# DanHelmy/hdr-realtime-video-pipeline

Hardware: AMD Instinct MI355X
Metric: frames/sec (HDRTVNet++ AGCM+LE+HG fp16 3840x2160 + fused RGB48 post into the pinned host ring); p50 per-frame ms in p50_ms (higher is better)
Workload: dtype f16

## Files before the change

### hdr-realtime-video-pipeline_amd/csrc/api_graph.hip

```cpp
#include "api.h"

namespace hdrtv_host {

void Seq::conv(const std::string &key, const f16 *src0, int c0, const f16 *src1, int c1, int Hi, int Wi, int act, int mode, f16 *dst, int dstC, int Hd, int Wd, const f16 *res1, const f16 *res2, f16 *dst_full, f16 *dst_planar, const f16 *res_planar, const float *dotw, float *dst_dot, int s0_stride)
{
    if (!ok()) return;
    auto it = c->conv.find(key);
    if (it == c->conv.end()) { rc = fail(c, HDRTV_ESTATE, "no packed conv %s", key.c_str()); return; }
    const ConvLayer &L = it->second;
    ConvParams p;
    memset(&p, 0, sizeof p);
    p.src0 = src0; p.src1 = src1; p.c0 = c0; p.c1 = c1;
    p.s0_stride = s0_stride ? s0_stride : c0; p.s1_stride = c1;
    p.Hi = Hi; p.Wi = Wi;
    const int pad = L.ks / 2;
    p.Ho = (Hi + 2 * pad - L.ks) / L.stride + 1;
    p.Wo = (Wi + 2 * pad - L.ks) / L.stride + 1;
    p.wpk = wtp<f16>(c, L.wpk); p.scale = wtp<float>(c, L.scale); p.shift = wtp<float>(c, L.shift);
    p.CoutPad = L.coutPad; p.Cout = L.cout; p.act = act; p.mode = mode;
    p.dst = dst; p.dst_full = dst_full; p.dstC = dstC; p.Hd = Hd; p.Wd = Wd;
    p.res1 = res1; p.res2 = res2; p.dst_planar = dst_planar; p.res_planar = res_planar;
    p.dotw = dotw; p.dst_dot = dst_dot;
    if (c0 + c1 != L.cin) { rc = fail(c, HDRTV_ESTATE, "conv %s: channel mismatch", key.c_str()); return; }
    p.zeros = wtp<f16>(c, c->zeros_off);
// ... 473 lines not shown
                q.chk(conv_c3_q8_launch(img, H, W, wtp<int8_t>(c, Lq.wpk8), wtp<float>(c, Lq.scale), wtp<float>(c, Lq.shift), Lq.q.inv(),
                                        Lq.q.zoff(), ACT_RELU, f0a, c->n_cu, q.s),
                      "LE.conv_first", "conv_c3_q8", (double)H * W * 27 * 32, (double)H * W * (6.0 + 64.0));
            }
            q.conv32("LE.HR_conv1", f0a, cond1, "LE.SFT_layer1", H, W, ACT_RELU, ST_NHWC, fea0, 32, H, W);
        } else {
            const bool fuse = !c->var.at("no_c3fuse") && !c->var.at("conv32_old") && c->q32.find("LE.HR_conv1") == c->q32.end();
            if (fuse) {
                q.conv32("LE.HR_conv1", f0a, cond1, "LE.SFT_layer1", H, W, ACT_RELU, ST_NHWC, fea0, 32, H, W, nullptr, nullptr, nullptr, nullptr,
                         img, "le.conv_first");
            } else {
                q.c3("le.conv_first", img, H, W, ACT_RELU, f0a, nullptr);
                q.conv32("LE.HR_conv1", f0a, cond1, "LE.SFT_layer1", H, W, ACT_RELU, ST_NHWC, fea0, 32, H, W);
            }
        }
    }
    f16 *fea1a = q.wsp<f16>("le.fea1a"), *fea1 = q.wsp<f16>("le.fea1"), *l1b = q.wsp<f16>("le.l1b");
    auto down = [&](const char *key, const f16 *src, int Hi, int Wi, f16 *dst, int Ho, int Wo) {
        if (isq8(key)) q.convq8(key, src, false, 32, Hi, Wi, ACT_RELU, dst, 32, nullptr);
        else q.conv(key, src, 32, nullptr, 0, Hi, Wi, ACT_RELU, ST_NHWC, dst, 32, Ho, Wo);
    };
    if (!head_fused) down("LE.down_conv1", fea0, H, W, fea1a, s.H1, s.W1);
    q.resblock("LE.recon_trunk1.0", fea1a, cond2, s.H1, s.W1, l1b, fea1);
    f16 *fea2a = q.wsp<f16>("le.fea2a"), *fea2 = q.wsp<f16>("le.fea2"), *l2b = q.wsp<f16>("le.l2b");
    down("LE.down_conv2", fea1, s.H1, s.W1, fea2a, s.H2, s.W2);
    q.resblock("LE.recon_trunk2.0", fea2a, cond3, s.H2, s.W2, l2b, fea2);
    f16 *fea3 = q.wsp<f16>("le.fea3"), *l3b = q.wsp<f16>("le.l3b"), *t3x = q.wsp<f16>("le.t3x"), *t3y = q.wsp<f16>("le.t3y");
    down("LE.down_conv3", fea2, s.H2, s.W2, fea3, s.H3, s.W3);
    q.resblock("LE.recon_trunk3.0", fea3, cond4, s.H3, s.W3, l3b, t3x);
    q.resblock("LE.recon_trunk3.1", t3x, cond4, s.H3, s.W3, l3b, t3y);
    q.resblock("LE.recon_trunk3.2", t3y, cond4, s.H3, s.W3, l3b, t3x);
    q.resblock("LE.recon_trunk3.3", t3x, cond4, s.H3, s.W3, l3b, t3y, fea3);
    f16 *up1 = q.wsp<f16>("le.up1"), *t4 = q.wsp<f16>("le.t4");
    q.conv32("LE.up_conv1.0", t3y, nullptr, "", s.H3, s.W3, ACT_RELU, ST_PS, up1, 32, s.H2, s.W2, fea2);
    q.resblock("LE.recon_trunk4.0", up1, cond3, s.H2, s.W2, l2b, t4);
    f16 *up2 = q.wsp<f16>("le.up2"), *t5 = q.wsp<f16>("le.t5");
    q.conv32("LE.up_conv2.0", t4, nullptr, "", s.H2, s.W2, ACT_RELU, ST_PS, up2, 32, s.H1, s.W1, fea1);
    q.resblock("LE.recon_trunk5.0", up2, cond2, s.H1, s.W1, l1b, t5);
    if (q.ok() && rows && c->var.at("le_rows_i8")) {
        auto qu = c->q32.find("LE.up_conv3.0"), qh = c->q32.find("LE.HR_conv2"), ql = c->q32.find("LE.conv_last");
        const SftLayer &S2 = c->sft.at("LE.SFT_layer2");
        if (qu != c->q32.end() && qh != c->q32.end() && ql != c->q32.end() && S2.q && qu->second.coutPad == 128 &&
            qh->second.coutPad == 32 && ql->second.coutPad == 32) {
            RowsTailI8Params p;
            memset(&p, 0, sizeof p);
            p.u = t5; p.fea0 = fea0; p.cond = cond1; p.res_planar = img; p.dst_planar = out_planar; p.H = H; p.W = W;
            p.up = q.rows_i8(qu->second); p.hr = q.rows_i8(qh->second); p.last = q.rows_i8(ql->second); p.s = q.rows_i8(S2);
            p.slope_relu = act_slope(ACT_RELU);
            p.trash = const_cast<char *>(wtp<char>(c, c->dump_off));
            const double npx = (double)H * W;
            q.chk(le_tail_rows_i8_launch(p, c->n_cu, q.s), "LE.tail", "le_tail_rows<i8>",
                  npx * (32.0 * 9 * 128 / 4 + 2.0 * (16 * 16 + 16 * 32) + 32.0 * 9 * 32 + 32.0 * 9 * 3), npx * (16 + 64 + 32 + 6 + 6) + 9.0 * 32 * (128 + 32 + 32));
            return q.rc;
        }
    }
    if (q.ok() && rows) {
        RowsTailParams p;
        memset(&p, 0, sizeof p);
        bool qu, qh, ql, qs;
        const ConvLayer *Lu = q.rows_conv("LE.up_conv3.0", p.fq_u, qu), *Lh = q.rows_conv("LE.HR_conv2", p.fq_y, qh),
                        *Ll = q.rows_conv("LE.conv_last", p.fq_z, ql);
        const SftLayer &S2 = c->sft.at("LE.SFT_layer2");
        if (Lu && Lh && Ll && q.rows_sft(S2, p.fq_s, qs)) {
            p.fq = (qu ? 1 : 0) | (qh ? 2 : 0) | (ql ? 4 : 0) | (qs ? 8 : 0);
            p.u = t5; p.fea0 = fea0; p.cond = cond1; p.res_planar = img; p.dst_planar = out_planar; p.H = H; p.W = W;
            p.w_up = wtp<f16>(c, Lu->wpk); p.b_up = wtp<float>(c, Lu->shift);
            p.sft_wfrag = wtp<f16>(c, S2.wfrag); p.sft_bias = wtp<float>(c, S2.bias);
            p.w_hr = wtp<f16>(c, Lh->wpk); p.b_hr = wtp<float>(c, Lh->shift); p.w_last = wtp<f16>(c, Ll->wpk); p.b_last = wtp<float>(c, Ll->shift);
            p.trash = const_cast<char *>(wtp<char>(c, c->dump_off));
            p.dump = q.stamp_buf();
            const double npx = (double)H * W;
            q.chk(le_tail_rows_launch(p, c->n_cu, q.s), "LE.tail", p.fq ? "le_tail_rows<fq>" : "le_tail_rows",
                  npx * (32.0 * 9 * 128 / 4 + 2.0 * (16 * 16 + 16 * 32) + 32.0 * 9 * 32 + 32.0 * 9 * 3), npx * (16 + 64 + 32 + 6 + 6) + 2.0 * 9 * 32 * (128 + 32 + 32));
            return q.rc;
        }
    }
    q.conv32("LE.up_conv3.0", t5, nullptr, "", s.H1, s.W1, ACT_RELU, ST_PS, up3, 32, H, W, fea0);
    q.conv32("LE.HR_conv2", up3, cond1, "LE.SFT_layer2", H, W, ACT_RELU, ST_NHWC, f0b, 32, H, W);
    q.conv32("LE.conv_last", f0b, nullptr, "", H, W, ACT_NONE, ST_PLANAR3, nullptr, 0, H, W, nullptr, nullptr, out_planar, img);
    return q.rc;
}

size_t hg_need_plan(hdrtv_ctx *c, int Hp, int Wp, HgNeedParams &p)
{
    memset(&p, 0, sizeof p);
    p.Hp = Hp; p.Wp = Wp;
    constexpr int n_layers = (int)(sizeof hg_layers / sizeof hg_layers[0]);
    static_assert(n_layers + 1 <= HG_NEED_MAX_LAYERS && n_layers + 3 <= HG_NEED_MAX_TENSORS, "hg_need's tables are too small");
    constexpr int max_level = [] { int m = 0; for (const HgLayer &L : hg_layers) m = L.level > m ? L.level : m; return m; }();
    static_assert(max_level < HG_NEED_LEVELS, "hg_need's unit tables have too few levels");
    memcpy(p.lu, hg_need_unit_log2[c->var.at("hg_sparse") == 1 ? 1 : 2], sizeof p.lu);
    auto ncell = [&](int level) { return (((Hp >> level) + 15) / 16) * (((Wp >> level) + 15) / 16); };
    auto nwords = [&](int level) {
        size_t m = 0;
        for (const auto &tab : hg_need_unit_log2) {
            const int u = 1 << tab[level], rows = std::max(((Hp >> level) + u - 1) / u, ((Hp >> level) + 7) / 8);
            m = std::max(m, (size_t)rows * ((((Wp >> level) + u - 1) / u + 63) / 64));
        }
        return m;
    };
    const char *names[HG_NEED_MAX_TENSORS];
    int level[HG_NEED_MAX_TENSORS], nt = 0;
    auto tensor = [&](const char *name, int lev) {
        if (!name) name = "part";
        for (int i = 0; i < nt; ++i)
            if (!strcmp(names[i], name)) return i;
        names[nt] = name; level[nt] = lev;
        return nt++;
    };
    for (int i = 0; i < n_layers; ++i) {
        const HgLayer &L = hg_layers[i];
        HgNeedLayer &N = p.L[i + 1];
        N.level = L.level; N.ks = L.ks; N.tw = 16;
        N.mode = L.mode == ST_POOL ? 1 : (L.ps ? 2 : 0);
        N.in = tensor(L.in, L.level);
        N.skip = L.skip ? tensor(L.skip, L.level) : -1;
        N.out = tensor(L.out, L.out_level());
        N.th = L.ks == 3 && Seq::prw_tile_rows(c, L.mode, L.cout, Hp >> L.level, Wp >> L.level) == 8 ? 8 : 16;
    }
    const int nt_table = nt;
    {
        HgNeedLayer &N = p.L[0];
        N.level = 0; N.ks = 3; N.mode = 1;
        N.out = tensor(hg_layers[0].in, 1);
        N.in = tensor("img", 0);
        N.skip = -1;
        N.th = 8; N.tw = 32;
    }
    p.n_layers = n_layers + 1;
    bool seen[HG_NEED_MAX_TENSORS] = {};
    for (int i = p.n_layers - 1; i >= 0; --i) {
        HgNeedLayer &N = p.L[i];
        N.in_first = !seen[N.in];
        seen[N.in] = true;
        if (N.skip >= 0) { N.skip_first = !seen[N.skip]; seen[N.skip] = true; }
    }
    size_t off = 0;
    auto take = [&](size_t bytes) { const size_t o = off; off = (off + bytes + 15) & ~(size_t)15; return (int)o; };
    p.flags_off = take((size_t)ncell(0));
    take((size_t)ncell(0));
    for (int t = 0; t < nt_table; ++t)
        if (strcmp(names[t], "part")) take((size_t)ncell(level[t]));
    for (int i = 1; i <= n_layers; ++i) p.L[i].list_off = take(4 * (2 * (size_t)ncell(p.L[i].level) + 4));
    size_t scratch = 0;
    for (int t = 0; t < nt; ++t) scratch = std::max(scratch, nwords(level[t]));
    for (int t = 0; t < nt_table; ++t) {
        p.map_off[t] = take(8 * nwords(level[t]));
        if (!strcmp(names[t], "part")) p.flags_map = t;
    }
    for (int i = 0; i < p.n_layers; ++i) {
        p.L[i].out_chained = i + 1 < p.n_layers ? p.L[i + 1].in == p.L[i].out : p.L[i].out == p.flags_map;
        p.L[i].in_chained = i > 0 && p.L[i - 1].out == p.L[i].in;
    }
    p.scratch_words = (int)scratch;
    p.kbits_off = take(8 * scratch);
    p.tbits_off = take(8 * scratch);
    p.L[0].list_off = take(4 * (2 * (size_t)ncell(0) + 4));
    p.map_off[nt_table] = take(8 * nwords(0));
    return off;
}

int run_hg(hdrtv_ctx *c, Seq &q, const f16 *base, void *out, int out_f32, bool complete_taps)
{
    const Shapes s = shapes_for(c->H, c->W);
    const int Hp = s.Hp, Wp = s.Wp;
    f16 *img = q.wsp<f16>("hg.img");
    uint8_t *mask = q.wsp<uint8_t>("hg.mask");
    const bool sparse = !complete_taps && c->var.at("hg_sparse") != 0 && !c->hg_i8 && !c->var.at("final_recompute");
    HgNeedParams np;
    if (sparse) {
        hg_need_plan(c, Hp, Wp, np);
        np.base = q.wsp<unsigned char>("hg.need");
    }
    if (q.ws == c->lane_ws[0] && !complete_taps) {
        hipStreamCaptureStatus cap = hipStreamCaptureStatusNone;
        c->taps_partial = sparse;
        c->taps_replayable = sparse && hipStreamIsCapturing(q.s, &cap) == hipSuccess && cap != hipStreamCaptureStatusNone;
        c->taps_stream = q.s;
    }
    if (!complete_taps)
        q.chk(hg_prep_launch(base, s.H, s.W, Hp, Wp, img, mask, c->mask_r, 0.1f, q.s, sparse ? np.base + np.flags_off : nullptr), "hg_prep",
              "hg_prep", 0.0, 13.0 * Hp * Wp);
    if (sparse) q.chk(hg_need_launch(np, q.s), "hg_need", "hg_need", 0.0, 0.0);
    float *part = q.wsp<float>("hg.part");
    const bool light = !c->var.at("final_recompute");
    float *part2 = light ? q.wsp<float>("hg.part2") : nullptr;
    const f16 *w2frag = light ? wtp<f16>(c, c->hgf_wfrag) + 6 * 64 * 8 : nullptr;
    constexpr int n_layers = (int)(sizeof hg_layers / sizeof hg_layers[0]);
    const char *tn[3 * n_layers];
    void *tp[3 * n_layers];
    int nt = 0;
    auto tensor = [&](const char *name) -> void * {
        if (!name) return nullptr;
        for (int i = 0; i < nt; ++i)
            if (!strcmp(tn[i], name)) return tp[i];
        char key[32];
        snprintf(key, sizeof key, "%s%s", c->hg_i8 ? "hg8." : "hg.", name);
        tn[nt] = name;
        tp[nt] = q.wsp<void>(key);
        return tp[nt++];
    };
    const bool c1_list = sparse && light;
    q.c3("hg.conv1", img, Hp, Wp, ACT_RELU, nullptr, (f16 *)tensor(hg_layers[0].in), c->hg_q0_inv, c->hg_q0_zero, w2frag, part2,
         c1_list ? reinterpret_cast<const int *>(np.base + np.L[0].list_off) : nullptr, c1_list ? ((Hp + 7) / 8) * ((Wp + 31) / 32) : 0);
    char key[32];
    for (const HgLayer &L : hg_layers) {
        snprintf(key, sizeof key, "hg.%s", L.name);
        if (sparse) {
            const HgNeedLayer &N = np.L[&L - hg_layers + 1];
            q.need_list = reinterpret_cast<const int *>(np.base + N.list_off);
            q.need_th = N.th;
            q.need_total = (((Hp >> L.level) + N.th - 1) / N.th) * (((Wp >> L.level) + 15) / 16);
        }
        const int c1 = L.skip_cin, c0 = L.cin - c1, Hi = Hp >> L.level, Wi = Wp >> L.level;
        const int Ho = Hp >> L.out_level(), Wo = Wp >> L.out_level();
        const bool dot3 = L.mode == ST_PS_DOT3;
        const float *dotw = dot3 ? wtp<float>(c, c->hg_w10a) : nullptr;
        float *dst_dot = dot3 ? part : nullptr;
        if (c->hg_i8)
            q.conv8(key, (const int8_t *)tensor(L.in), c0, (const int8_t *)tensor(L.skip), c1, Hi, Wi, L.mode, tensor(L.out), L.out_c(), Ho, Wo, dotw, dst_dot);
        else
            q.conv(key, (const f16 *)tensor(L.in), c0, (const f16 *)tensor(L.skip), c1, Hi, Wi, L.act, L.mode, (f16 *)tensor(L.out), L.out_c(), Ho, Wo,
                   nullptr, nullptr, nullptr, nullptr, nullptr, dotw, dst_dot);
    }
    if (!q.ok() || complete_taps) return q.rc;
    const C3Layer &L1 = c->c3.at("hg.conv1");
    HgFinalFusedArgs fa;
    fa.img = img; fa.mask = mask; fa.part = part; fa.wfrag = wtp<f16>(c, c->hgf_wfrag);
    fa.scale = wtp<float>(c, L1.scale); fa.shift = wtp<float>(c, L1.shift);
    fa.b10 = wtp<float>(c, c->f32v.at("hg.b10"));
    fa.wl = wtp<float>(c, c->f32v.at("hg.wl")); fa.bl = wtp<float>(c, c->f32v.at("hg.bl"));
    fa.out = out; fa.out_f32 = out_f32; fa.H = s.H; fa.W = s.W; fa.Hp = Hp; fa.Wp = Wp;
    if (light)
        q.chk(hg_final_light_launch(fa, part2, q.s), "hg_final", "hg_final_light", (double)s.H * s.W * 6 * 3,
              (double)s.H * s.W * (6 + 1 + 32 + 3 * (out_f32 ? 4 : 2)));
#ifdef HDRTV_AB
    else
        q.chk(hg_final_fused_launch(fa, c->n_cu, q.s), "hg_final", "hg_final_fused", (double)Hp * Wp * (128 * 3 + 6 * 3),
              (double)s.H * s.W * (6 + 1 + 16 + 3 * (out_f32 ? 4 : 2)));
#endif
    return q.rc;
}

}
```

### hdr-realtime-video-pipeline_amd/csrc/api_util.hip

```cpp
#include "api.h"

namespace hdrtv_host {

int fail(hdrtv_ctx *c, int code, const char *fmt, ...)
{
    char buf[512];
    va_list ap;
    va_start(ap, fmt);
    vsnprintf(buf, sizeof buf, fmt, ap);
    va_end(ap);
    if (c) { std::lock_guard<std::mutex> lk(c->err_mu); c->err = buf; }
    return code;
}

namespace {
const std::pair<const char *, int> k_variants[] = {
    {"le_rows", 1},
    {"le_rows_min", 8},
    {"le_rows_i8", 1},
    {"le_rows_fq", 1},
    {"prw", 1},
    {"prw_i8", 1},
    {"pglds_nt_slow", 3},
    {"no_t16", 0},
    {"conv32_old", 0},
    {"conv32_nosplit", 0},
    {"conv32_nw", 0},
    {"no_c3fuse", 0},
    {"no_c3q8", 0},
    {"glds1_old", 0},
    {"hg_sparse", 2},
    {"final_recompute", 0},
    {"cond3_fused", 1},
    {"cond2_fused", 1},
    {"pre_split", 0},
    {"force_ncu", 0},
    {"light_wgs", 2},
    {"fs_passes", 3},
    {"f32_narrow_below", 0},
    {"f32_mfma", 1},
};
const char *const k_ab_only[] = {"conv32_old", "conv32_nosplit", "conv32_nw", "glds1_old", "final_recompute"};
}
bool variant_allowed(const std::string &name, int value)
{
#ifdef HDRTV_AB
    (void)name; (void)value;
    return true;
#else
    if (value == 0) return true;
    for (const char *n : k_ab_only) if (name == n) return false;
    return true;
#endif
}
void variants_init(hdrtv_ctx *c)
{
    for (const auto &kv : k_variants) c->var[kv.first] = kv.second;
    const char *e = getenv("HDRTV_VARIANTS");
    if (!e) return;
    std::string str(e);
    size_t pos = 0;
    while (pos < str.size()) {
        size_t nx = str.find(',', pos);
        if (nx == std::string::npos) nx = str.size();
        const std::string one = str.substr(pos, nx - pos);
        const size_t eq = one.find('=');
        if (eq != std::string::npos) {
            auto it = c->var.find(one.substr(0, eq));
            if (it != c->var.end() && variant_allowed(it->first, atoi(one.c_str() + eq + 1))) it->second = atoi(one.c_str() + eq + 1);
        }
        pos = nx + 1;
    }
}

}
```

### hdr-realtime-video-pipeline_amd/csrc/hg_need.hip

```cpp
#include "launchers.h"

namespace {

constexpr int NT = 1024, LDS_WORDS = 2304;
using u64 = unsigned long long;

__constant__ u64 k_tile_bits[5] = {~0ull, 0x5555555555555555ull, 0x1111111111111111ull, 0x0101010101010101ull, 0x0001000100010001ull};

struct Map {
    int h, w, nw;
};
__device__ __forceinline__ Map map_of(const HgNeedParams &p, int level)
{
    const int lu = p.lu[level], r = (1 << lu) - 1;
    Map m;
    m.h = ((p.Hp >> level) + r) >> lu;
    m.w = ((p.Wp >> level) + r) >> lu;
    m.nw = (m.w + 63) >> 6;
    return m;
}
__device__ __forceinline__ u64 word(const u64 *b, const Map &m, int y, int wi)
{
    return (unsigned)y < (unsigned)m.h && (unsigned)wi < (unsigned)m.nw ? b[y * m.nw + wi] : 0;
}
__device__ __forceinline__ u64 row_mask(int w, int wi)
{
    const int n = w - 64 * wi;
    return n >= 64 ? ~0ull : (n <= 0 ? 0ull : (1ull << n) - 1);
}
__device__ __forceinline__ u64 spread2(unsigned v)
{
    u64 x = v;
    x = (x | x << 16) & 0x0000FFFF0000FFFFull;
    x = (x | x << 8) & 0x00FF00FF00FF00FFull;
    x = (x | x << 4) & 0x0F0F0F0F0F0F0F0Full;
    x = (x | x << 2) & 0x3333333333333333ull;
    x = (x | x << 1) & 0x5555555555555555ull;
    return x | x << 1;
}
__device__ __forceinline__ unsigned pairs_any(u64 v)
{
    u64 x = (v | v >> 1) & 0x5555555555555555ull;
    x = (x | x >> 1) & 0x3333333333333333ull;
    x = (x | x >> 2) & 0x0F0F0F0F0F0F0F0Full;
    x = (x | x >> 4) & 0x00FF00FF00FF00FFull;
    x = (x | x >> 8) & 0x0000FFFF0000FFFFull;
    x = (x | x >> 16) & 0x00000000FFFFFFFFull;
    return (unsigned)x;
}

__global__ __launch_bounds__(NT) void hg_need_kernel(HgNeedParams p)
{
    __shared__ u64 s_k[LDS_WORDS], s_t[LDS_WORDS], s_n[LDS_WORDS];
    __shared__ int s_wave[NT / 64];
    const int tid = threadIdx.x;
    {
        const Map m = map_of(p, 0);
        const HgNeedLayer &L = p.L[p.n_layers - 1];
        u64 *fb = L.out_chained && m.h * m.nw <= LDS_WORDS ? s_n : reinterpret_cast<u64 *>(p.base + p.map_off[p.flags_map]);
        unsigned char *fl = p.base + p.flags_off;
        constexpr int NW = NT / 64, B = 8;
        const int lane = tid & 63, n0 = m.h * m.nw;
        for (int i0 = tid >> 6; i0 < n0; i0 += B * NW) {
            int at[B];
            unsigned char c[B];
#pragma unroll
            for (int j = 0; j < B; ++j) {
                const int i = i0 + j * NW, y = i / m.nw, x = 64 * (i - y * m.nw) + lane;
                at[j] = i < n0 && x < m.w ? y * m.w + x : -1;
                c[j] = at[j] >= 0 ? fl[at[j]] : 0;
            }
#pragma unroll
            for (int j = 0; j < B; ++j) {
                const u64 v = __ballot(c[j] != 0);
                if (at[j] >= 0) fl[at[j]] = 0;
                if (lane == 0 && i0 + j * NW < n0) fb[i0 + j * NW] = v;
            }
        }
    }
    __syncthreads();
    for (int li = p.n_layers - 1; li >= 0; --li) {
        const HgNeedLayer L = p.L[li];
        const int olev = L.level + (L.mode == 1 ? 1 : 0) - (L.mode == 2 ? 1 : 0);
        const Map mk = map_of(p, L.level), mo = map_of(p, olev);
        const int lu = p.lu[L.level], nk = mk.h * mk.nw;
        const int sh = p.lu[olev] - lu + olev - L.level;
        const int lth = L.th == 8 ? 3 : 4, ltw = L.tw == 32 ? 5 : 4, lbw = ltw - lu;
        const int ty_n = ((p.Hp >> L.level) + L.th - 1) >> lth, tx_n = ((p.Wp >> L.level) + (1 << ltw) - 1) >> ltw, nt = ty_n * mk.nw;
        const bool lds = max(nk, nt) <= LDS_WORDS;
        u64 *km = lds ? s_k : reinterpret_cast<u64 *>(p.base + p.kbits_off);
        u64 *tm = lds ? s_t : reinterpret_cast<u64 *>(p.base + p.tbits_off);
        const u64 *om = L.out_chained && mo.h * mo.nw <= LDS_WORDS ? s_n : reinterpret_cast<const u64 *>(p.base + p.map_off[L.out]);
        for (int i = tid; i < nk; i += NT) {
            const int y = i / mk.nw, wi = i - y * mk.nw;
            u64 k;
            if (sh == 0) {
                k = word(om, mo, y, wi);
            } else if (sh > 0) {
                k = spread2((unsigned)(word(om, mo, y >> 1, wi >> 1) >> (32 * (wi & 1))));
            } else {
                k = 0;
                for (int dy = 0; dy < 2; ++dy)
                    k |= (u64)pairs_any(word(om, mo, 2 * y + dy, 2 * wi)) | (u64)pairs_any(word(om, mo, 2 * y + dy, 2 * wi + 1)) << 32;
            }
            km[i] = k & row_mask(mk.w, wi);
        }
        __syncthreads();
        u64 *ig = reinterpret_cast<u64 *>(p.base + p.map_off[L.in]), *im = L.in_chained && nk <= LDS_WORDS ? s_n : ig;
        u64 *sm = L.skip >= 0 ? reinterpret_cast<u64 *>(p.base + p.map_off[L.skip]) : nullptr;
        for (int i = tid; i < nk; i += NT) {
            const int y = i / mk.nw, wi = i - y * mk.nw;
            u64 v = km[i];
            if (L.ks == 3) {
                for (int dy = -1; dy <= 1; ++dy) {
                    const u64 c = word(km, mk, y + dy, wi);
                    v |= c | c << 1 | c >> 1 | word(km, mk, y + dy, wi - 1) >> 63 | word(km, mk, y + dy, wi + 1) << 63;
                }
                v &= row_mask(mk.w, wi);
            }
            im[i] = L.in_first ? v : (ig[i] | v);
            if (sm) sm[i] = L.skip_first ? v : (sm[i] | v);
        }
        const int r_sh = lth - lu;
        for (int i = tid; i < nt; i += NT) {
            const int ty = i / mk.nw, wi = i - ty * mk.nw;
            const int r0 = r_sh >= 0 ? ty << r_sh : ty >> -r_sh, nr = r_sh >= 0 ? 1 << r_sh : 1;
            u64 v = 0;
            for (int r = r0; r < min(r0 + nr, mk.h); ++r) v |= km[r * mk.nw + wi];
            for (int s = 1; s < (1 << lbw); s <<= 1) v |= v >> s;
            tm[i] = v & k_tile_bits[lbw];
        }
        __syncthreads();
        const int per = (nt + NT - 1) / NT, c0 = tid * per, c1 = min(nt, c0 + per);
        int cnt = 0;
        for (int i = c0; i < c1; ++i) cnt += __popcll(tm[i]);
        int incl = cnt;
        for (int d = 1; d < 64; d <<= 1) {
            const int v = __shfl_up(incl, d, 64);
            if ((tid & 63) >= d) incl += v;
        }
        if ((tid & 63) == 63) s_wave[tid >> 6] = incl;
        __syncthreads();
        int o = incl - cnt, total = 0;
        for (int w = 0; w < NT / 64; ++w) {
            const int v = s_wave[w];
            if (w < (tid >> 6)) o += v;
            total += v;
        }
        int *lst = reinterpret_cast<int *>(p.base + L.list_off);
        if (tid == 0) lst[0] = total;
        for (int i = c0; i < c1; ++i) {
            const int ty = i / mk.nw, wi = i - ty * mk.nw;
            for (u64 v = tm[i]; v; v &= v - 1) lst[1 + o++] = ty * tx_n + ((64 * wi + __ffsll(v) - 1) >> lbw);
        }
    }
}

}

hipError_t hg_need_launch(const HgNeedParams &p, hipStream_t s)
{
    if (!p.base || p.n_layers < 1 || p.n_layers > HG_NEED_MAX_LAYERS) return hipErrorInvalidValue;
    for (int i = 0; i < p.n_layers; ++i) {
        const HgNeedLayer &L = p.L[i];
        const int olev = L.level + (L.mode == 1 ? 1 : 0) - (L.mode == 2 ? 1 : 0);
        if (L.level < 0 || L.level >= HG_NEED_LEVELS || olev < 0 || olev >= HG_NEED_LEVELS) return hipErrorInvalidValue;
        const int sh = p.lu[olev] - p.lu[L.level] + olev - L.level;
        if (p.lu[L.level] < 0 || p.lu[L.level] > 4 || sh < -1 || sh > 1 || (L.th != 8 && L.th != 16) ||
            (L.tw != 0 && L.tw != 16 && L.tw != 32))
            return hipErrorInvalidValue;
    }
    if (p.lu[0] != 4) return hipErrorInvalidValue;
    hipLaunchKernelGGL(hg_need_kernel, dim3(1), dim3(NT), 0, s, p);
    return hipGetLastError();
}
```

### hdr-realtime-video-pipeline_amd/csrc/launchers.h

```cpp
#pragma once
#include "common.h"

struct DevOnce {
    unsigned char set[64] = {};
    static int cur() { int d = 0; return hipGetDevice(&d) == hipSuccess && d >= 0 && d < 64 ? d : 0; }
    bool need() const { return !set[cur()]; }
    void done() { set[cur()] = 1; }
};
template <class K> hipError_t allow_lds(DevOnce &once, K kern, int bytes)
{
    if (!once.need()) return hipSuccess;
    const hipError_t e = hipFuncSetAttribute(reinterpret_cast<const void *>(kern), hipFuncAttributeMaxDynamicSharedMemorySize, bytes);
    if (e == hipSuccess) once.done();
    return e;
}

hipError_t conv_igemm_launch(ConvParams p, int cin_t, int bn, int ks, int stride, hipStream_t stream);
hipError_t conv_glds1_launch(ConvParams p, hipStream_t stream, int n_cu = 0, bool old_form = false, bool *list_taken = nullptr);
hipError_t conv_pglds_launch(ConvParams p, int n_cu, hipStream_t stream, bool *list_taken = nullptr);
hipError_t conv_prw_launch(ConvParams p, int th, int n_cu, hipStream_t stream, bool *list_taken = nullptr);
hipError_t conv_pglds_i8_launch(ConvI8Params p, int n_cu, hipStream_t stream);
hipError_t conv_prw_i8_launch(ConvI8Params p, int th, int n_cu, hipStream_t stream);
hipError_t conv1x1_i8_launch(ConvI8Params p, hipStream_t stream);
hipError_t conv32p_launch(Conv32Params p, int n_cu, hipStream_t stream, int nw = 0);
hipError_t conv32s_launch(Conv32Params p, int n_cu, hipStream_t stream, bool nosplit = false);
hipError_t le_rb_rows_launch(RowsRbParams p, int n_cu, hipStream_t stream);
hipError_t le_rb_rows_i8_launch(RowsRbI8Params p, int n_cu, hipStream_t stream);
hipError_t le_tail_rows_i8_launch(RowsTailI8Params p, int n_cu, hipStream_t stream);
hipError_t le_head_rows_i8_launch(RowsHeadI8Params p, int n_cu, hipStream_t stream);
hipError_t le_tail_rows_launch(RowsTailParams p, int n_cu, hipStream_t stream);
hipError_t le_head_rows_launch(RowsHeadParams p, int n_cu, hipStream_t stream);
hipError_t conv_t16_launch(ConvParams p, hipStream_t stream, int n_cu);
hipError_t conv_q8_launch(ConvQ8Params p, hipStream_t stream, int n_cu);
hipError_t conv_q8_multi_launch(ConvQ8MultiParams p, int n_cu, hipStream_t stream);
hipError_t conv3x3s2_preg_launch(ConvParams p, int n_cu, hipStream_t stream);

hipError_t pre_unpack_launch(const uint8_t *bgr, f16 *out, int H, int W, hipStream_t s);
struct AaTables {
    const float *wx;
    const int *xmn, *xns;
    const float *wy;
    const int *ymn, *yns;
};
hipError_t cond_resize_launch(const f16 *in, f16 *out, int H, int W, int Ho, int Wo, const AaTables &t, hipStream_t s);
hipError_t pre_fused_launch(const uint8_t *bgr, f16 *out, f16 *cond, int H, int W, int Ho, int Wo, const AaTables &t, int mode, hipStream_t s);
hipError_t post_u8_launch(const void *in, int is_f32, int H, int W, uint8_t *bgr, hipStream_t s);
hipError_t post_rgb48_launch(const void *in, int is_f32, int H, int W, uint16_t *rgb, int pq, float peak, hipStream_t s,
                             const float *pq_bnd = nullptr);

struct FakeQ { int on; float inv, zoff, scale, zero; };
hipError_t cls_block_launch(const void *in, int in_f16, int Ci, int Hi, int Wi, const float *nmean, const float *nrstd,
                            const float *ngamma, const float *nbeta, const float *Wt, const float *bias, int Co, float *out,
                            int Ho, int Wo, float *part, hipStream_t s, const FakeQ *qin = nullptr, const FakeQ *qstat = nullptr,
                            int *nblk = nullptr);
hipError_t cls_stats_launch(const float *part, int C, int nblk, int n, float eps, float *mean, float *rstd, hipStream_t s);
struct AgcmFoldArgs {
    const float *mean5;
    const float *w20, *b20;
    const float *ws[3], *bs[3], *wt[3], *bt[3];
    const float *w1, *b1, *w2, *b2, *w3, *b3;
};
hipError_t agcm_fold_launch(const AgcmFoldArgs &a, f16 *frags, float *biasbuf, hipStream_t s);
hipError_t agcm_mlp_launch(const f16 *in, f16 *out, size_t npix, const f16 *frags, const float *biasbuf, hipStream_t s);

hipError_t conv_c3_launch(const f16 *in, int H, int W, const f16 *wfrag, const float *scale, const float *shift, int cout,
                          int act, f16 *out, f16 *out_pool, int n_cu, hipStream_t s, float pool_q_inv = 0.f, float pool_q_zero = 0.f,
                          const f16 *w2frag = nullptr, float *part2 = nullptr,
                          const int *tile_list = nullptr, bool *list_taken = nullptr);
hipError_t conv_c3_q8_launch(const f16 *in, int H, int W, const int8_t *wq, const float *scale, const float *shift, float q_inv,
                             float q_zoff, int act, f16 *out, int n_cu, hipStream_t s);
struct QLastArgs {
    const int8_t *wq;
    const float *ss;
    float q_inv, q_zoff;
};
hipError_t le_cond_trunk_launch(const f16 *img, int H, int W, const f16 *wfrag, const float *bias, f16 *cond, f16 *cond1,
                                int n_cu, hipStream_t s, const QLastArgs *q6 = nullptr);
hipError_t cond_tail_launch(const f16 *x, int x_stride, size_t npx, const f16 *wfrag, const float *bias, f16 *out, int n_cu,
                            hipStream_t s, const QLastArgs *q2 = nullptr);
struct TrunkQ8Args {
    const int8_t *wfrag;
    const float *consts;
    float q1_inv, q1_zoff, q4_inv;
    float zoff[5];
};
hipError_t le_cond_trunk_q8_launch(const f16 *img, int H, int W, const TrunkQ8Args &a, f16 *cond, f16 *cond1, int n_cu, hipStream_t s);
hipError_t cond_tail_q8_launch(const int8_t *x, size_t npx, const int8_t *wfrag, const float *consts, float zoff2, f16 *out, int n_cu,
                               hipStream_t s);
hipError_t agcm_mlp_q8_launch(const f16 *in, f16 *out, size_t npix, const int8_t *wfrag, const float *consts, float q1_inv, float q1_zoff,
                              float zoff2, float zoff3, hipStream_t s);
hipError_t planar3_to_q8_launch(const f16 *in, size_t npix, float inv, float zoff, int8_t *out, hipStream_t s);
struct AgcmFoldQ8Args {
    FakeQ q20, qlin[6];
    const float *P, *Q;
    float inv2, inv3;
    float *consts;
};
hipError_t agcm_fold_q8_launch(const AgcmFoldArgs &a, const AgcmFoldQ8Args &q, float *biasbuf, hipStream_t s);
hipError_t hg_prep_launch(const f16 *base, int H, int W, int Hp, int Wp, f16 *img_pad, uint8_t *mask, float r, float thresh,
                          hipStream_t s, uint8_t *flags = nullptr);
constexpr int HG_NEED_MAX_LAYERS = 24, HG_NEED_MAX_TENSORS = 32, HG_NEED_LEVELS = 6;
constexpr int hg_need_unit_log2[3][HG_NEED_LEVELS] = {{4, 4, 4, 4, 4, 4}, {4, 4, 4, 4, 4, 4}, {4, 2, 1, 0, 0, 0}};
struct HgNeedLayer {
    int level, mode, ks;
    int in, skip, out;
    int in_first, skip_first;
    int out_chained;
    int in_chained;
    int th, tw;
    int list_off;
};
struct HgNeedParams {
    unsigned char *base;
    int Hp, Wp, n_layers;
    int lu[HG_NEED_LEVELS];
    int flags_off;
    int flags_map;
    int kbits_off, tbits_off, scratch_words;
    int map_off[HG_NEED_MAX_TENSORS];
    HgNeedLayer L[HG_NEED_MAX_LAYERS];
};
hipError_t hg_need_launch(const HgNeedParams &p, hipStream_t s);
struct HgFinalFusedArgs {
    const f16 *img;
    const uint8_t *mask;
    const float *part;
    const f16 *wfrag;
    const float *scale, *shift, *b10, *wl, *bl;
    void *out;
    int out_f32, H, W, Hp, Wp;
};
hipError_t hg_final_fused_launch(const HgFinalFusedArgs &a, int n_cu, hipStream_t s);
hipError_t hg_final_light_launch(const HgFinalFusedArgs &a, const float *part2, hipStream_t s);
hipError_t letterbox_launch(const LetterboxParams &p, hipStream_t s);
hipError_t post_scale_launch(const PostScaleParams &p, int is_f32, int pq, hipStream_t s);
hipError_t post_scale_ar_launch(const PostScaleParams &p, int antiring, int is_f32, int pq, hipStream_t s);
hipError_t post_scale_cas_launch(const PostScaleParams &p, int antiring, int cas, int is_f32, int pq, hipStream_t s);
hipError_t post_fsr_launch(const PostFsrParams &p, int rcas, float sharp, int is_f32, int pq, hipStream_t s);
hipError_t film_grain_launch(const uint16_t *src, uint16_t *dst, int H, int W, float intensity, float seed, hipStream_t s);
hipError_t post_rgb48_grain_launch(const void *in, int is_f32, int H, int W, uint16_t *rgb, int pq, float peak, const float *pq_bnd,
                                   float intensity, float seed, hipStream_t s);
hipError_t post_scale_grain_launch(const PostScaleParams &p, int antiring, int cas, float intensity, float seed, int is_f32, int pq,
                                   hipStream_t s);
hipError_t post_fsr_grain_launch(const PostFsrParams &p, int rcas, float sharp, float intensity, float seed, int is_f32, int pq, hipStream_t s);
hipError_t post_down_launch(const PostDownParams &p, int antiring, int ssim, int is_f32, int pq, hipStream_t s);
hipError_t post_ssimsr_launch(const PostSsimsrParams &p, int ssim, int is_f32, int pq, hipStream_t s);
hipError_t post_ycbcr10_launch(const Ycbcr10Params &p, int is_f32, int pq, hipStream_t s);
hipError_t rgb48_to_ycbcr10_launch(const Ycbcr10Params &p, hipStream_t s);
hipError_t post_ycbcr10_dither_launch(const Ycbcr10Params &p, int is_f32, int pq, hipStream_t s);
hipError_t rgb48_to_ycbcr10_dither_launch(const Ycbcr10Params &p, hipStream_t s);
int64_t ycbcr10_fs_scratch_bytes(int fmt, int H, int W);
hipError_t post_ycbcr10_fs_launch(const Ycbcr10Params &p, int is_f32, int pq, void *scratch, int passes, hipStream_t s);
hipError_t rgb48_to_ycbcr10_fs_launch(const Ycbcr10Params &p, void *scratch, int passes, hipStream_t s);
hipError_t rgb48_deband_launch(const DebandParams &p, hipStream_t s);
hipError_t light_stats_launch(const LightStatsParams &p, int is_f32, int pq, int max_wgs, hipStream_t s);
hipError_t rgb48_light_stats_launch(const LightStatsParams &p, int max_wgs, hipStream_t s);
hipError_t metrics_launch(const MetricsParams &p, hipStream_t s);
int metrics_blocks(int H, int W);
hipError_t metrics_u16_launch(const MetricsParams &p, hipStream_t s);
hipError_t border_counts_launch(const BorderCountsParams &p, hipStream_t s);
bool area_reduce_size_ok(int sh, int sw, int nh, int nw);
hipError_t area_reduce_launch(const AreaReduceParams &p, hipStream_t s);
hipError_t channel_hist_launch(const ChannelHistParams &p, hipStream_t s);
void grade_match_host(const uint32_t *hist, double n, float peak_nits, float *out12);

hipError_t conv_f32_launch(const F32ConvParams &p, int ks, int stride, int n_cu, hipStream_t s);
bool conv_f32_on_mfma(const F32ConvParams &p, int ks, int n_cu);
hipError_t ew_f32_launch(int op, const float *a, const float *b, const float *c, float *y, size_t n, hipStream_t s);
hipError_t avgpool3s2_leaky_f32_launch(const float *x, float *y, int C, int H, int W, float slope, hipStream_t s);
hipError_t instnorm_f32_launch(float *x, const float *gamma, const float *beta, int C, int n, float eps, hipStream_t s);
hipError_t plane_mean_f32_launch(const float *x, float *y, int C, int n, hipStream_t s);
hipError_t gfm_heads_f32_launch(const F32GfmParams &p, hipStream_t s);
hipError_t maxpool2_f32_launch(const float *x, float *y, int C, int H, int W, hipStream_t s);
hipError_t window_f32_launch(const float *x, float *y, int C, int H, int W, int Ho, int Wo, int mode, hipStream_t s);
hipError_t hg_mask_f32_launch(const float *base, float *mask, size_t npix, float r, hipStream_t s);
hipError_t hg_blend_f32_launch(const float *t, const float *img, const float *mask, float *out, int H, int W, int Hp, int Wp,
                               hipStream_t s);
hipError_t pre_f32_launch(const uint8_t *bgr, float *rgb, float *cond, int H, int W, int Ho, int Wo, const AaTables &t, int mode, hipStream_t s);
hipError_t cond_resize_f32_launch(const float *rgb, float *cond, int H, int W, int Ho, int Wo, const AaTables &t, int mode, hipStream_t s);
```

Baseline: 149.5.

## Speed up HG need-planning kernel with LDS-resident maps and early exits

Rewrites the single-workgroup hg_need kernel so that, when every layer's bitmaps fit, all maps including skip maps stay in LDS, using lighter barriers. Adds fast paths: return immediately when no flags are set, and stop propagating when a layer's need mask is full, emitting dense tile lists for the remaining layers. The list compaction changes from a per-thread serial scan to wave-parallel ballot-based emission, and the flag gather runs with larger unrolling. This targets the latency of a serial one-block planning kernel, at the cost of more complexity and more LDS.

```diff
diff --git a/hdr-realtime-video-pipeline_amd/csrc/api_graph.hip b/hdr-realtime-video-pipeline_amd/csrc/api_graph.hip
--- a/hdr-realtime-video-pipeline_amd/csrc/api_graph.hip
+++ b/hdr-realtime-video-pipeline_amd/csrc/api_graph.hip
@@ -649,6 +649,7 @@
         p.L[i].out_chained = i + 1 < p.n_layers ? p.L[i + 1].in == p.L[i].out : p.L[i].out == p.flags_map;
         p.L[i].in_chained = i > 0 && p.L[i - 1].out == p.L[i].in;
     }
+    p.fast = c->var.at("hg_need_fast") != 0;
     p.scratch_words = (int)scratch;
     p.kbits_off = take(8 * scratch);
     p.tbits_off = take(8 * scratch);
diff --git a/hdr-realtime-video-pipeline_amd/csrc/api_util.hip b/hdr-realtime-video-pipeline_amd/csrc/api_util.hip
--- a/hdr-realtime-video-pipeline_amd/csrc/api_util.hip
+++ b/hdr-realtime-video-pipeline_amd/csrc/api_util.hip
@@ -30,6 +30,7 @@
     {"no_c3q8", 0},
     {"glds1_old", 0},
     {"hg_sparse", 2},
+    {"hg_need_fast", 1},
     {"final_recompute", 0},
     {"cond3_fused", 1},
     {"cond2_fused", 1},
diff --git a/hdr-realtime-video-pipeline_amd/csrc/hg_need.hip b/hdr-realtime-video-pipeline_amd/csrc/hg_need.hip
--- a/hdr-realtime-video-pipeline_amd/csrc/hg_need.hip
+++ b/hdr-realtime-video-pipeline_amd/csrc/hg_need.hip
@@ -2,7 +2,8 @@
 
 namespace {
 
-constexpr int NT = 1024, LDS_WORDS = 2304;
+constexpr int NT = 1024, NWAVE = NT / 64, LDS_WORDS = 2304, SKIP_SLOTS = 4;
+constexpr int LDS_BYTES = 3 * LDS_WORDS * 8, LDS_BYTES_ALL = (3 + SKIP_SLOTS) * LDS_WORDS * 8;
 using u64 = unsigned long long;
 
 __constant__ u64 k_tile_bits[5] = {~0ull, 0x5555555555555555ull, 0x1111111111111111ull, 0x0101010101010101ull, 0x0001000100010001ull};
@@ -10,7 +11,7 @@
 struct Map {
     int h, w, nw;
 };
-__device__ __forceinline__ Map map_of(const HgNeedParams &p, int level)
+__host__ __device__ __forceinline__ Map map_of(const HgNeedParams &p, int level)
 {
     const int lu = p.lu[level], r = (1 << lu) - 1;
     Map m;
@@ -18,6 +19,19 @@
     m.w = ((p.Wp >> level) + r) >> lu;
     m.nw = (m.w + 63) >> 6;
     return m;
+}
+__host__ __device__ __forceinline__ int out_level(const HgNeedLayer &L) { return L.level + (L.mode == 1 ? 1 : 0) - (L.mode == 2 ? 1 : 0); }
+struct Tiles {
+    int lth, ltw, ty_n, tx_n;
+};
+__host__ __device__ __forceinline__ Tiles tiles_of(const HgNeedParams &p, const HgNeedLayer &L)
+{
+    Tiles t;
+    t.lth = L.th == 8 ? 3 : 4;
+    t.ltw = L.tw == 32 ? 5 : 4;
+    t.ty_n = ((p.Hp >> L.level) + L.th - 1) >> t.lth;
+    t.tx_n = ((p.Wp >> L.level) + (1 << t.ltw) - 1) >> t.ltw;
+    return t;
 }
 __device__ __forceinline__ u64 word(const u64 *b, const Map &m, int y, int wi)
 {
@@ -48,49 +62,74 @@
     x = (x | x >> 16) & 0x00000000FFFFFFFFull;
     return (unsigned)x;
 }
-
-__global__ __launch_bounds__(NT) void hg_need_kernel(HgNeedParams p)
-{
-    __shared__ u64 s_k[LDS_WORDS], s_t[LDS_WORDS], s_n[LDS_WORDS];
-    __shared__ int s_wave[NT / 64];
-    const int tid = threadIdx.x;
+template <bool ALL> __device__ __forceinline__ void chain_barrier()
+{
+    if constexpr (ALL) {
+        __builtin_amdgcn_fence(__ATOMIC_RELEASE, "workgroup", "local");
+        __builtin_amdgcn_s_barrier();
+        __builtin_amdgcn_fence(__ATOMIC_ACQUIRE, "workgroup", "local");
+    } else {
+        __syncthreads();
+    }
+}
+
+template <bool ALL> __global__ __launch_bounds__(NT) void hg_need_kernel(HgNeedParams p)
+{
+    extern __shared__ u64 s_maps[];
+    u64 *const s_k = s_maps, *const s_t = s_maps + LDS_WORDS, *const s_n = s_maps + 2 * LDS_WORDS, *const s_skip = s_maps + 3 * LDS_WORDS;
+    __shared__ int s_wave[NWAVE], s_any[NWAVE], s_full[NWAVE];
+    const int tid = threadIdx.x, lane = tid & 63, wave = tid >> 6;
     {
         const Map m = map_of(p, 0);
         const HgNeedLayer &L = p.L[p.n_layers - 1];
-        u64 *fb = L.out_chained && m.h * m.nw <= LDS_WORDS ? s_n : reinterpret_cast<u64 *>(p.base + p.map_off[p.flags_map]);
+        u64 *fb = ALL || (L.out_chained && m.h * m.nw <= LDS_WORDS) ? s_n : reinterpret_cast<u64 *>(p.base + p.map_off[p.flags_map]);
         unsigned char *fl = p.base + p.flags_off;
-        constexpr int NW = NT / 64, B = 8;
-        const int lane = tid & 63, n0 = m.h * m.nw;
-        for (int i0 = tid >> 6; i0 < n0; i0 += B * NW) {
+        constexpr int B = 16;
+        const int n0 = m.h * m.nw;
+        u64 any = 0;
+        for (int i0 = wave; i0 < n0; i0 += B * NWAVE) {
             int at[B];
             unsigned char c[B];
 #pragma unroll
             for (int j = 0; j < B; ++j) {
-                const int i = i0 + j * NW, y = i / m.nw, x = 64 * (i - y * m.nw) + lane;
+                const int i = i0 + j * NWAVE, y = i / m.nw, x = 64 * (i - y * m.nw) + lane;
                 at[j] = i < n0 && x < m.w ? y * m.w + x : -1;
-                c[j] = at[j] >= 0 ? fl[at[j]] : 0;
+                c[j] = fl[max(at[j], 0)];
             }
 #pragma unroll
             for (int j = 0; j < B; ++j) {
-                const u64 v = __ballot(c[j] != 0);
+                const u64 v = __ballot(at[j] >= 0 && c[j] != 0);
+                any |= v;
                 if (at[j] >= 0) fl[at[j]] = 0;
-                if (lane == 0 && i0 + j * NW < n0) fb[i0 + j * NW] = v;
-            }
-        }
-    }
-    __syncthreads();
-    for (int li = p.n_layers - 1; li >= 0; --li) {
+                if (lane == 0 && i0 + j * NWAVE < n0) fb[i0 + j * NWAVE] = v;
+            }
+        }
+        if (lane == 0) s_any[wave] = any != 0;
+    }
+    chain_barrier<ALL>();
+    if (p.fast) {
+        int any = 0;
+        for (int w = 0; w < NWAVE; ++w) any |= s_any[w];
+        if (!any) {
+            if (tid == 0)
+                for (int l = 0; l < p.n_layers; ++l) *reinterpret_cast<int *>(p.base + p.L[l].list_off) = 0;
+            return;
+        }
+    }
+    int li = p.n_layers - 1;
+    for (; li >= 0; --li) {
         const HgNeedLayer L = p.L[li];
-        const int olev = L.level + (L.mode == 1 ? 1 : 0) - (L.mode == 2 ? 1 : 0);
+        const int olev = out_level(L);
         const Map mk = map_of(p, L.level), mo = map_of(p, olev);
         const int lu = p.lu[L.level], nk = mk.h * mk.nw;
         const int sh = p.lu[olev] - lu + olev - L.level;
-        const int lth = L.th == 8 ? 3 : 4, ltw = L.tw == 32 ? 5 : 4, lbw = ltw - lu;
-        const int ty_n = ((p.Hp >> L.level) + L.th - 1) >> lth, tx_n = ((p.Wp >> L.level) + (1 << ltw) - 1) >> ltw, nt = ty_n * mk.nw;
-        const bool lds = max(nk, nt) <= LDS_WORDS;
+        const Tiles T = tiles_of(p, L);
+        const int lth = T.lth, lbw = T.ltw - lu, ty_n = T.ty_n, tx_n = T.tx_n, nt = ty_n * mk.nw;
+        const bool lds = ALL || max(nk, nt) <= LDS_WORDS;
         u64 *km = lds ? s_k : reinterpret_cast<u64 *>(p.base + p.kbits_off);
         u64 *tm = lds ? s_t : reinterpret_cast<u64 *>(p.base + p.tbits_off);
-        const u64 *om = L.out_chained && mo.h * mo.nw <= LDS_WORDS ? s_n : reinterpret_cast<const u64 *>(p.base + p.map_off[L.out]);
+        const u64 *om = ALL || (L.out_chained && mo.h * mo.nw <= LDS_WORDS) ? s_n : reinterpret_cast<const u64 *>(p.base + p.map_off[L.out]);
+        bool full = true;
         for (int i = tid; i < nk; i += NT) {
             const int y = i / mk.nw, wi = i - y * mk.nw;
             u64 k;
@@ -103,11 +142,24 @@
                 for (int dy = 0; dy < 2; ++dy)
                     k |= (u64)pairs_any(word(om, mo, 2 * y + dy, 2 * wi)) | (u64)pairs_any(word(om, mo, 2 * y + dy, 2 * wi + 1)) << 32;
             }
-            km[i] = k & row_mask(mk.w, wi);
-        }
-        __syncthreads();
-        u64 *ig = reinterpret_cast<u64 *>(p.base + p.map_off[L.in]), *im = L.in_chained && nk <= LDS_WORDS ? s_n : ig;
-        u64 *sm = L.skip >= 0 ? reinterpret_cast<u64 *>(p.base + p.map_off[L.skip]) : nullptr;
+            const u64 rm = row_mask(mk.w, wi);
+            km[i] = k & rm;
+            full = full && (k & rm) == rm;
+        }
+        {
+            const u64 not_full = __ballot(!full);
+            if (lane == 0) s_full[wave] = not_full == 0;
+        }
+        chain_barrier<ALL>();
+        if (p.fast) {
+            int all_full = 1;
+            for (int w = 0; w < NWAVE; ++w) all_full &= s_full[w];
+            if (all_full) break;
+        }
+        u64 *ig = reinterpret_cast<u64 *>(p.base + p.map_off[L.in]);
+        u64 *im = (ALL ? L.in_chained : L.in_chained && nk <= LDS_WORDS) ? s_n : ig;
+        u64 *sm = L.skip < 0 ? nullptr : (ALL ? s_skip + p.lds_slot[L.skip] * LDS_WORDS : reinterpret_cast<u64 *>(p.base + p.map_off[L.skip]));
+        const u64 *ip = L.in_first ? nullptr : (ALL ? s_skip + p.lds_slot[L.in] * LDS_WORDS : ig);
         for (int i = tid; i < nk; i += NT) {
             const int y = i / mk.nw, wi = i - y * mk.nw;
             u64 v = km[i];
@@ -118,7 +170,7 @@
                 }
                 v &= row_mask(mk.w, wi);
             }
-            im[i] = L.in_first ? v : (ig[i] | v);
+            im[i] = ip ? (ip[i] | v) : v;
             if (sm) sm[i] = L.skip_first ? v : (sm[i] | v);
         }
         const int r_sh = lth - lu;
@@ -130,30 +182,61 @@
             for (int s = 1; s < (1 << lbw); s <<= 1) v |= v >> s;
             tm[i] = v & k_tile_bits[lbw];
         }
-        __syncthreads();
-        const int per = (nt + NT - 1) / NT, c0 = tid * per, c1 = min(nt, c0 + per);
+        chain_barrier<ALL>();
+        const int wper = (((nt + NWAVE - 1) / NWAVE + (1 << lbw) - 1) >> lbw) << lbw, c0 = min(nt, wave * wper), c1 = min(nt, c0 + wper);
         int cnt = 0;
-        for (int i = c0; i < c1; ++i) cnt += __popcll(tm[i]);
-        int incl = cnt;
-        for (int d = 1; d < 64; d <<= 1) {
-            const int v = __shfl_up(incl, d, 64);
-            if ((tid & 63) >= d) incl += v;
-        }
-        if ((tid & 63) == 63) s_wave[tid >> 6] = incl;
-        __syncthreads();
-        int o = incl - cnt, total = 0;
-        for (int w = 0; w < NT / 64; ++w) {
+        for (int i = c0 + lane; i < c1; i += 64) cnt += __popcll(tm[i]);
+        for (int d = 32; d >= 1; d >>= 1) cnt += __shfl_xor(cnt, d, 64);
+        if (lane == 0) s_wave[wave] = cnt;
+        chain_barrier<ALL>();
+        int o = 0, total = 0;
+        for (int w = 0; w < NWAVE; ++w) {
             const int v = s_wave[w];
-            if (w < (tid >> 6)) o += v;
+            if (w < wave) o += v;
             total += v;
         }
         int *lst = reinterpret_cast<int *>(p.base + L.list_off);
         if (tid == 0) lst[0] = total;
-        for (int i = c0; i < c1; ++i) {
-            const int ty = i / mk.nw, wi = i - ty * mk.nw;
-            for (u64 v = tm[i]; v; v &= v - 1) lst[1 + o++] = ty * tx_n + ((64 * wi + __ffsll(v) - 1) >> lbw);
-        }
-    }
+        const int lsl = 6 - lbw;
+        for (int s0 = c0 << lsl; s0 < (c1 << lsl) && cnt; s0 += 64) {
+            const int s = s0 + lane, i = s >> lsl, bit = (s & ((1 << lsl) - 1)) << lbw;
+            const bool on = i < c1 && (tm[i] >> bit & 1);
+            const u64 b = __ballot(on);
+            if (on) {
+                const int ty = i / mk.nw, wi = i - ty * mk.nw;
+                lst[1 + o + __popcll(b & ((1ull << lane) - 1))] = ty * tx_n + ((64 * wi + bit) >> lbw);
+            }
+            o += __popcll(b);
+        }
+    }
+    for (; li >= 0; --li) {
+        const HgNeedLayer &L = p.L[li];
+        const Tiles T = tiles_of(p, L);
+        const int n = T.ty_n * T.tx_n;
+        int *lst = reinterpret_cast<int *>(p.base + L.list_off);
+        if (tid == 0) lst[0] = n;
+        for (int i = tid; i < n; i += NT) lst[1 + i] = i;
+    }
+}
+
+bool plan_lds(HgNeedParams &p)
+{
+    for (int &s : p.lds_slot) s = -1;
+    const Map m0 = map_of(p, 0);
+    if (m0.h * m0.nw > LDS_WORDS) return false;
+    int slots = 0;
+    for (int i = p.n_layers - 1; i >= 0; --i) {
+        const HgNeedLayer &L = p.L[i];
+        const Map mk = map_of(p, L.level), mo = map_of(p, out_level(L));
+        if (std::max(mk.h * mk.nw, tiles_of(p, L).ty_n * mk.nw) > LDS_WORDS || mo.h * mo.nw > LDS_WORDS) return false;
+        if (!L.out_chained || (i > 0 && !L.in_chained)) return false;
+        if (L.skip >= 0 && p.lds_slot[L.skip] < 0) {
+            if (!L.skip_first || slots == SKIP_SLOTS) return false;
+            p.lds_slot[L.skip] = slots++;
+        }
+        if (!L.in_first && p.lds_slot[L.in] < 0) return false;
+    }
+    return true;
 }
 
 }
@@ -163,14 +246,23 @@
     if (!p.base || p.n_layers < 1 || p.n_layers > HG_NEED_MAX_LAYERS) return hipErrorInvalidValue;
     for (int i = 0; i < p.n_layers; ++i) {
         const HgNeedLayer &L = p.L[i];
-        const int olev = L.level + (L.mode == 1 ? 1 : 0) - (L.mode == 2 ? 1 : 0);
+        const int olev = out_level(L);
         if (L.level < 0 || L.level >= HG_NEED_LEVELS || olev < 0 || olev >= HG_NEED_LEVELS) return hipErrorInvalidValue;
         const int sh = p.lu[olev] - p.lu[L.level] + olev - L.level;
         if (p.lu[L.level] < 0 || p.lu[L.level] > 4 || sh < -1 || sh > 1 || (L.th != 8 && L.th != 16) ||
             (L.tw != 0 && L.tw != 16 && L.tw != 32))
             return hipErrorInvalidValue;
+        if (L.in < 0 || L.in >= HG_NEED_MAX_TENSORS || L.skip >= HG_NEED_MAX_TENSORS || L.out < 0 || L.out >= HG_NEED_MAX_TENSORS)
+            return hipErrorInvalidValue;
     }
     if (p.lu[0] != 4) return hipErrorInvalidValue;
-    hipLaunchKernelGGL(hg_need_kernel, dim3(1), dim3(NT), 0, s, p);
+    HgNeedParams q = p;
+    if (plan_lds(q)) {
+        static DevOnce once;
+        if (hipError_t e = allow_lds(once, hg_need_kernel<true>, LDS_BYTES_ALL)) return e;
+        hipLaunchKernelGGL(hg_need_kernel<true>, dim3(1), dim3(NT), LDS_BYTES_ALL, s, q);
+    } else {
+        hipLaunchKernelGGL(hg_need_kernel<false>, dim3(1), dim3(NT), LDS_BYTES, s, q);
+    }
     return hipGetLastError();
 }
diff --git a/hdr-realtime-video-pipeline_amd/csrc/launchers.h b/hdr-realtime-video-pipeline_amd/csrc/launchers.h
--- a/hdr-realtime-video-pipeline_amd/csrc/launchers.h
+++ b/hdr-realtime-video-pipeline_amd/csrc/launchers.h
@@ -118,6 +118,8 @@
     int flags_map;
     int kbits_off, tbits_off, scratch_words;
     int map_off[HG_NEED_MAX_TENSORS];
+    int fast;
+    int lds_slot[HG_NEED_MAX_TENSORS];
     HgNeedLayer L[HG_NEED_MAX_LAYERS];
 };
 hipError_t hg_need_launch(const HgNeedParams &p, hipStream_t s);
```

Result: no change. 150.6 (median of 6 runs) (+0.7%).
